# theouterlimitz/Audio-Mastering-Engine

Measured on AMD Instinct MI355X. Metric: mastered Msamples/sec (48 kHz stereo f32) at 1/2/4/8 GPUs; % HBM roofline, higher is better.
Workload: dtype f64

## Files before the change

### audio-mastering-engine_amd/csrc/amx_dyn.hip

```cpp
#include "amx_dev.hpp"

namespace amx {

typedef double d2v __attribute__((ext_vector_type(2)));
typedef uint32_t u4v __attribute__((ext_vector_type(4)));

#define AMX_TAB 32769

#define AMX_RMS_N 4096
#define AMX_RMS_MAXLOOK 1024

__device__ __forceinline__ int rms_slot(int k) { return k + (k >> 4); }

__device__ __forceinline__ uint32_t rms_floor(uint64_t S, uint32_t cnt, double rc) {
    const double sd = fma((double)(uint32_t)(S >> 32), 4294967296.0, (double)(uint32_t)S);
    const double cd = (double)cnt;
    const uint32_t k = (uint32_t)__builtin_amdgcn_sqrtf((float)(sd * rc));
    const uint32_t k1 = k + 1;
    const bool up = (double)__umul24(k1, k1) * cd <= sd;
    const bool down = (double)__umul24(k, k) * cd > sd;
    const uint32_t r = k + (uint32_t)up - (uint32_t)(down & !up);
    return cnt ? (r > 32768u ? 32768u : r) : 0u;
}

#ifndef AMX_RMS_N256
#define AMX_RMS_N256 4096
#endif
template <int LP, int N>
__global__ void __launch_bounds__(AMX_BLOCK) k_rms(const ChainDev *__restrict__ cdp,
                                                   const ChunkDev *__restrict__ chunks,
                                                   const uint32_t *__restrict__ bands,
                                                   uint16_t *__restrict__ mi, int64_t nloc,
                                                   int *bact) {
    constexpr int F = N - LP;
    constexpr int PER = N / AMX_BLOCK;
    constexpr int VEC = PER / 4;
    static_assert(F % AMX_BLOCK == 0 && PER % 4 == 0, "tile shape");
    __shared__ unsigned long long P[N + N / 16];
    __shared__ unsigned long long wsum[AMX_BLOCK / 64];
    const int look = cdp->look;
    const int c = blockIdx.y, b = blockIdx.z;
    const ChunkDev ch = chunks[c];
    const int64_t base = (int64_t)blockIdx.x * F;
    if (base >= ch.n) return;
    const uint32_t *x = bands + b * nloc + ch.loc_off;
    uint16_t *mo = mi + b * nloc + ch.loc_off;
    const int64_t rowlen = (ch.n + 15) / 16 * 16;
    const int64_t f0 = base - LP;
    const int t = threadIdx.x;
    uint32_t v[PER];
    if (f0 >= 0 && f0 + N <= ch.n) {
#pragma unroll
        for (int q = 0; q < VEC; q++) {
            const u4v u = *reinterpret_cast<const u4v *>(x + f0 + t * PER + 4 * q);
#pragma unroll
            for (int e = 0; e < 4; e++) {
                const int32_t a0 = lo16(u[e]), a1 = hi16(u[e]);
                v[4 * q + e] = (uint32_t)(a0 * a0) + (uint32_t)(a1 * a1);
            }
        }
    } else {
#pragma unroll
        for (int q = 0; q < VEC; q++) {
            const int64_t f = f0 + t * PER + 4 * q;
            const bool ok = f >= 0 && f < rowlen;
            const u4v u = *reinterpret_cast<const u4v *>(x + (ok ? f : 0));
#pragma unroll
            for (int e = 0; e < 4; e++) {
                const int32_t a0 = lo16(u[e]), a1 = hi16(u[e]);
                v[4 * q + e] = (ok && f + e < ch.n) ? (uint32_t)(a0 * a0) + (uint32_t)(a1 * a1) : 0u;
            }
        }
    }
    unsigned long long run = 0;
#pragma unroll
    for (int q = 0; q < PER; q++) run += v[q];
    unsigned long long incl = run;
    const int lane = t & 63, w = t >> 6;
#pragma unroll
    for (int o = 1; o < 64; o <<= 1) {
        const unsigned long long up = __shfl_up(incl, o);
        if (lane >= o) incl += up;
    }
    if (lane == 63) wsum[w] = incl;
    __syncthreads();
    unsigned long long p = incl - run;
    for (int q = 0; q < w; q++) p += wsum[q];
    const int s0 = rms_slot(t * PER);
#pragma unroll
    for (int q = 0; q < PER; q++) { p += v[q]; P[s0 + q] = p; }
    __syncthreads();
    constexpr int OUT = F / AMX_BLOCK;
    const uint32_t cfull = 2u * (uint32_t)look;
    const double rfull = 1.0 / (double)cfull;
    const bool whole = base >= look && base + F <= ch.n;
    auto rms_at = [&](int k) -> uint32_t {
        const uint32_t nn = (uint32_t)t + (uint32_t)k * AMX_BLOCK;
        const uint32_t e1 = nn + (LP - 1), e0 = e1 - (uint32_t)look;
        const uint64_t S = P[e1 + (e1 >> 4)] - P[e0 + (e0 >> 4)];
        if (whole) return rms_floor(S, cfull, rfull);
        const int64_t i = base + nn;
        const bool head = i < look;
        const uint32_t cnt = head ? 2u * (uint32_t)i : cfull;
        return rms_floor(S, cnt, head ? 1.0 / (double)cnt : rfull);
    };
    const uint32_t rq = (uint32_t)cdp->rq[b];
    bool hot = false;
    if (whole) {
#pragma unroll
        for (int k = 0; k < OUT; k++) {
            const uint32_t rms = rms_at(k);
            hot |= rms >= rq;
            mo[base + t + k * AMX_BLOCK] = (uint16_t)rms;
        }
    } else {
#pragma unroll
        for (int k = 0; k < OUT; k++) {
            const int64_t i = base + t + k * AMX_BLOCK;
            const uint32_t rms = rms_at(k);
            hot |= i < ch.n && rms >= rq;
            if (i < rowlen) mo[i] = i < ch.n ? (uint16_t)rms : (uint16_t)0;
        }
    }
    if (__syncthreads_or(hot) && t == 0 && bact[b] == 0) bact[b] = 1;
}

__device__ __forceinline__ double m_of(const double *__restrict__ mt, uint32_t r) {
    return mt[r < 32768u ? r : 32768u];
}


template <bool RCP>
__device__ __forceinline__ double env_div(double m, double a, double ra) {
    if constexpr (RCP) {
        const double q = m * ra;
        return fma(fma(-q, a, m), ra, q);
    } else {
        return m / a;
    }
}

__device__ __forceinline__ double min_f64_raw(double a, double b) {
    double r;
    asm("v_min_f64 %0, %1, %2" : "=v"(r) : "v"(a), "v"(b));
    return r;
}

__device__ __forceinline__ double env_step3(double att, double m, double inc, double dec) {
    const double up = min_f64_raw(att + inc, m);
    const double dn = fmax(att - dec, 0.0);
    return att <= m ? up : dn;
}

template <bool RCP>
__device__ __forceinline__ double env_step(const ChainDev &cd, double att, double m) {
    return env_step3(att, m, env_div<RCP>(m, cd.env_A, cd.env_rA), env_div<RCP>(m, cd.env_R, cd.env_rR));
}

__device__ __forceinline__ int mul16(int v, double f) {
    return (int)floor((double)v * f);
}

__device__ __forceinline__ double exp10_gain(const double *__restrict__ E, double x) {
    const double k = rint(x * E[0]);
    double r = fma(E[1], k, x);
    r = fma(E[2], k, r);
    double u = r * E[3];
    u = fma(E[4], r, u);
    double p = fma(E[5], u, E[6]);
#pragma unroll
    for (int i = 7; i < 15; i++) p = fma(u, p, E[i]);
    p = fma(u, p, 1.0);
    p = fma(u, p, 1.0);
    return ldexp(p, (int)k);
}

__device__ __forceinline__ double gain_factor(const ChainDev &cd, double att) {
    const double q = -att * cd.exc[15];
    return exp10_gain(cd.exc, fma(fma(-q, 20.0, -att), cd.exc[15], q));
}

__device__ __forceinline__ uint32_t gain_apply(uint32_t v, double f) {
    return pack2((int16_t)mul16(lo16(v), f), (int16_t)mul16(hi16(v), f));
}

__device__ __forceinline__ uint32_t gain_frame(const ChainDev &cd, uint32_t v, double att) {
    return gain_apply(v, gain_factor(cd, att));
}

#define AMX_ENV_TF_ 16

__device__ __forceinline__ double lane_val(double v, int i) {
    const long long x = __double_as_longlong(v);
    const int lo = __builtin_amdgcn_readlane((int)x, i);
    const int hi = __builtin_amdgcn_readlane((int)(x >> 32), i);
    return __longlong_as_double(((long long)hi << 32) | (unsigned)lo);
}

template <bool RCP>
__device__ double env_rerun_wave(const ChainDev &cd, const uint16_t *m, const double *mt, double *ckr,
                                 int64_t f0, int64_t f1, double ns, double old_end) {
    __shared__ __attribute__((aligned(16))) double s_m[64], s_i[64], s_d[64];
    const int lane = threadIdx.x & 63;
    const bool ckl = (lane & (AMX_ENV_TF_ - 1)) == 0;
    double c = ns;
    auto ridx = [&](int64_t f) -> uint32_t { return f < f1 ? (uint32_t)m[f] : 0xffffffffu; };
    auto gath = [&](uint32_t r) -> double { return r == 0xffffffffu ? 0.0 : m_of(mt, r); };
    auto ckld = [&](int64_t f) -> double { return ckl && f < f1 ? ckr[f / AMX_ENV_TF_] : 0.0; };
    double ml = gath(ridx(f0 + lane));
    uint32_t ib = ridx(f0 + 128 + lane);
    double m1 = gath(ridx(f0 + 64 + lane));
    double ol = ckld(f0 + lane), o1 = ckld(f0 + 64 + lane);
    for (int64_t base = f0; base < f1; base += 64) {
        const uint32_t ic = ridx(base + 192 + lane);
        const double m2 = gath(ib);
        const double o2 = ckld(base + 128 + lane);
        s_m[lane] = ml;
        s_i[lane] = env_div<RCP>(ml, cd.env_A, cd.env_rA);
        s_d[lane] = env_div<RCP>(ml, cd.env_R, cd.env_rR);
        __builtin_amdgcn_fence(__ATOMIC_SEQ_CST, "wavefront");
        __builtin_amdgcn_wave_barrier();
        double mine = c;
        int stop = 4;
#pragma unroll
        for (int t = 0; t < 4; t++) {
            double mv[16], iv[16], dv[16];
#pragma unroll
            for (int q = 0; q < 16; q += 2) {
                const d2v a = *reinterpret_cast<const d2v *>(s_m + 16 * t + q);
                const d2v b = *reinterpret_cast<const d2v *>(s_i + 16 * t + q);
                const d2v d = *reinterpret_cast<const d2v *>(s_d + 16 * t + q);
                mv[q] = a.x; mv[q + 1] = a.y;
                iv[q] = b.x; iv[q + 1] = b.y;
                dv[q] = d.x; dv[q + 1] = d.y;
            }
            const bool same = base + 16 * t < f1 && c == lane_val(ol, 16 * t);
            if (__builtin_amdgcn_readfirstlane((int)same)) { stop = t; break; }
            mine = lane == 16 * t ? c : mine;
#pragma unroll
            for (int q = 0; q < 16; q++) c = env_step3(c, mv[q], iv[q], dv[q]);
        }
        __builtin_amdgcn_wave_barrier();
        if (ckl && (lane >> 4) < stop && base + lane < f1) ckr[(base + lane) / AMX_ENV_TF_] = mine;
        if (stop < 4) return old_end;
        ml = m1;
        m1 = m2;
        ib = ic;
        ol = o1;
        o1 = o2;
    }
    return c;
}

struct EnvBands {
    int mask;
    int nb;
    __device__ __forceinline__ bool act(int b) const { return (mask >> b) & 1; }
};
__device__ __forceinline__ EnvBands env_bands(const int *bact) {
    EnvBands e;
    e.mask = 0;
#pragma unroll
    for (int b = 0; b < 3; b++) e.mask |= (__builtin_amdgcn_readfirstlane(bact[b]) != 0) << b;
    e.nb = __builtin_popcount(e.mask);
    return e;
}
__device__ __forceinline__ int env_slot_band(const EnvBands &e, int s) {
    int m = e.mask;
    for (int k = 0; k < s; k++) m &= m - 1;
    return __builtin_ctz(m | 8);
}

#define AMX_ENV_TF 16
#define AMX_ENV_MP 18
#define AMX_ENV_PF 8

typedef uint32_t u2v __attribute__((ext_vector_type(2)));

__device__ __forceinline__ void env_gather(const double *__restrict__ mt, const u2v (&I)[4],
                                           double (&G)[16]) {
#pragma unroll
    for (int i = 0; i < 4; i++) {
#pragma unroll
        for (int e = 0; e < 4; e++) {
            const uint32_t r = (I[i][e >> 1] >> (16 * (e & 1))) & 0xffffu;
            G[4 * i + e] = mt[r];
        }
    }
}

template <bool RCP>
__device__ __forceinline__ void env0_tile(const ChainDev &cd, double *sm, double (&G)[16],
                                          u2v (&Islot)[4], const u2v (&Inext)[4],
                                          const uint16_t *const (&irow)[4], const double *mt, int q,
                                          int ntile, int nwarm, int64_t start, int64_t end,
                                          double *ckr, double &att, double &s_spec, bool &any) {
    const int lane = threadIdx.x & 63;
#pragma unroll
    for (int i = 0; i < 4; i++) {
        double *d = sm + ((lane >> 2) + 16 * i) * AMX_ENV_MP + 4 * (lane & 3);
        *reinterpret_cast<d2v *>(d) = d2v{G[4 * i], G[4 * i + 1]};
        *reinterpret_cast<d2v *>(d + 2) = d2v{G[4 * i + 2], G[4 * i + 3]};
    }
    __builtin_amdgcn_wave_barrier();
    {
        const int qn = (q + AMX_ENV_PF < ntile ? q + AMX_ENV_PF : q) * AMX_ENV_TF;
#pragma unroll
        for (int i = 0; i < 4; i++) Islot[i] = *reinterpret_cast<const u2v *>(irow[i] + qn);
        env_gather(mt, Inext, G);
    }
    const int64_t f0 = start + (int64_t)q * AMX_ENV_TF;
    const bool in = f0 >= 0 && f0 < end;
    double mv[AMX_ENV_TF];
#pragma unroll
    for (int i = 0; i < 8; i++) {
        const d2v v = *reinterpret_cast<const d2v *>(sm + lane * AMX_ENV_MP + 2 * i);
        mv[2 * i] = v.x;
        mv[2 * i + 1] = v.y;
    }
    __builtin_amdgcn_wave_barrier();
    if (q == nwarm) s_spec = att;
    if (in) {
        if (q >= nwarm) {
            ckr[f0 / AMX_ENV_TF] = att;
            uint32_t h = 0, l = 0;
#pragma unroll
            for (int f = 0; f < AMX_ENV_TF; f++) {
                const unsigned long long x = (unsigned long long)__double_as_longlong(mv[f]);
                h |= (uint32_t)(x >> 32);
                l |= (uint32_t)x;
            }
            any |= ((h & 0x7fffffffu) | l) != 0u;
        }
        double iv[AMX_ENV_TF], dv[AMX_ENV_TF];
#pragma unroll
        for (int f = 0; f < AMX_ENV_TF; f++) {
            iv[f] = env_div<RCP>(mv[f], cd.env_A, cd.env_rA);
            dv[f] = env_div<RCP>(mv[f], cd.env_R, cd.env_rR);
        }
#pragma unroll
        for (int f = 0; f < AMX_ENV_TF; f++) att = env_step3(att, mv[f], iv[f], dv[f]);
    }
}

#define AMX_ENV_WG 4
#define AMX_ENV_LDS_PIN (48 * 1024)
template <bool RCP>
__global__ void __launch_bounds__(64 * AMX_ENV_WG) k_env0(const ChainDev *__restrict__ cdp,
                                             const ChunkDev *__restrict__ chunks,
                                             const SegDev *__restrict__ es, int n_es,
                                             const uint16_t *__restrict__ mi,
                                             const double *__restrict__ tabs,
                                             double *__restrict__ ck,
                                             double *__restrict__ sv, double *__restrict__ ev,
                                             int *__restrict__ act, int64_t nloc, int warm,
                                             int *__restrict__ flags) {
    __shared__ __attribute__((aligned(16))) double sm_all[AMX_ENV_WG][64 * AMX_ENV_MP];
    const ChainDev &cd = *cdp;
    const int lane = threadIdx.x & 63, wv = __builtin_amdgcn_readfirstlane(threadIdx.x >> 6);
    double *sm = sm_all[wv];
    if (blockIdx.x == 0 && blockIdx.y == 0 && threadIdx.x < AMX_ENV_MAX_ROUNDS) flags[threadIdx.x] = 0;
    if (blockIdx.x == 0 && blockIdx.y == 0 && threadIdx.x < 64) {
        for (int k = lane; k < AMX_ENV_MAX_ROUNDS * AMX_ENV_NCTR; k += 64) flags[AMX_ENV_MAX_ROUNDS + k] = 0;
        if (lane < 3) flags[AMX_ENV_LIST + lane] = 0;
    }
    const EnvBands eb = env_bands(flags + AMX_ENV_BACT);
    if ((int)blockIdx.y >= eb.nb) return;
    const int b = env_slot_band(eb, blockIdx.y);
    es += cd.etab[eb.nb].es_off;
    n_es = cd.etab[eb.nb].n_es;
    const int Le = cd.etab[eb.nb].Le, ld = cd.es_ld;
    if ((int)(blockIdx.x * (blockDim.x >> 6)) * 64 >= n_es) return;
    const int j = (blockIdx.x * (blockDim.x >> 6) + wv) * 64 + lane;
    const bool valid = j < n_es;
    const SegDev sg = es[valid ? j : n_es - 1];
    const ChunkDev ch = chunks[sg.chunk];
    const int64_t rowoff = b * nloc + ch.loc_off;
    const int64_t start = sg.pos - warm;
    const int64_t end = valid ? sg.pos + sg.len : sg.pos;
    double *ckr = ck + rowoff / AMX_ENV_TF;
    const double *mt = tabs + (int64_t)b * 3 * AMX_TAB;
    const int ntile = (warm + Le) / AMX_ENV_TF, nwarm = warm / AMX_ENV_TF;
    const uint16_t *irow[4];
#pragma unroll
    for (int i = 0; i < 4; i++) {
        const int r = 16 * i + (lane >> 2);
        irow[i] = mi + __shfl(rowoff + start, r) + 4 * (lane & 3);
    }
    u2v I[AMX_ENV_PF][4];
#pragma unroll
    for (int u = 0; u < AMX_ENV_PF; u++)
#pragma unroll
        for (int i = 0; i < 4; i++) I[u][i] = *reinterpret_cast<const u2v *>(irow[i] + u * AMX_ENV_TF);
    double G[2][16];
    env_gather(mt, I[0], G[0]);
    env_gather(mt, I[1], G[1]);
    double att = 0.0, s_spec = 0.0;
    if (cd.env_guess && start >= 0) att = mt[mi[rowoff + start]];
    bool any = false;
    for (int q0 = 0; q0 < ntile; q0 += AMX_ENV_PF) {
#pragma unroll
        for (int u = 0; u < AMX_ENV_PF; u++)
            env0_tile<RCP>(cd, sm, G[u & 1], I[u], I[(u + 2) % AMX_ENV_PF], irow, mt,
                           q0 + u, ntile, nwarm, start, end, ckr, att, s_spec, any);
    }
    if (valid) {
        sv[(int64_t)b * ld + j] = s_spec;
        ev[(int64_t)b * ld + j] = att;
        act[(int64_t)b * ld + j] = any ? 1 : 0;
    }
}

template <bool RCP>
__device__ __forceinline__ double env_fix_segment(const ChainDev &cd, const uint16_t *mrow,
                                                  const double *mt, double *ckr, int64_t pos, int len,
                                                  bool active, double ns, double old_end) {
    if (!active) {
        const int64_t k0 = pos / AMX_ENV_TF_, k1 = (pos + len + AMX_ENV_TF_ - 1) / AMX_ENV_TF_;
        for (int64_t k = k0 + (threadIdx.x & 63); k < k1; k += 64) ckr[k] = ns;
        return ns;
    }
    return env_rerun_wave<RCP>(cd, mrow, mt, ckr, pos, pos + len, ns, old_end);
}

template <bool RCP>
__global__ void __launch_bounds__(64) k_envneed(const ChainDev *__restrict__ cdp,
                                                const SegDev *__restrict__ es, int n_es,
                                                const double *__restrict__ sv,
                                                const double *__restrict__ ev,
                                                const int *__restrict__ act, int *flags,
                                                int *__restrict__ prev, int *__restrict__ list) {
    const ChainDev &cd = *cdp;
    const int b = blockIdx.y, lane = threadIdx.x;
    const EnvBands eb = env_bands(flags + AMX_ENV_BACT);
    if (!eb.act(b)) return;
    es += cd.etab[eb.nb].es_off;
    n_es = cd.etab[eb.nb].n_es;
    const int w0 = blockIdx.x * 64;
    if (w0 >= n_es) return;
    const int j = w0 + lane;
    const bool valid = j < n_es;
    const int64_t bo = (int64_t)b * cd.es_ld;
    const SegDev sg = es[valid ? j : n_es - 1];
    const bool a = valid && act[bo + j] != 0;
    const unsigned long long am = __ballot(a);
    const unsigned long long below = lane ? am & (~0ull >> (64 - lane)) : 0ull;
    int p = below ? w0 + 63 - __clzll((long long)below) : -1;
    if (p < sg.first) p = -1;
    const bool lb = valid && p < 0 && sg.first < w0;
    if (__ballot(lb)) {
        const int first0 = __shfl(sg.first, 0);
        int last = -1;
        for (int base = w0 - 64; base + 63 >= first0; base -= 64) {
            const int jj = base + lane;
            const unsigned long long mk = __ballot(jj >= first0 && act[bo + jj] != 0);
            if (mk) { last = base + 63 - __clzll((long long)mk); break; }
        }
        if (lb) p = last;
    }
    bool need = false;
    if (valid) {
        prev[bo + j] = p;
        need = !((p >= 0 ? ev[bo + p] : 0.0) == sv[bo + j]);
    }
    const unsigned long long nm = __ballot(need);
    if (nm) {
        int base = 0;
        if (lane == 0) base = atomicAdd(flags + AMX_ENV_LIST, __popcll(nm));
        base = __shfl(base, 0);
        const unsigned long long lt = lane ? ~0ull >> (64 - lane) : 0ull;
        if (need) list[base + __popcll(nm & lt)] = (int)(bo + j);
    }
}

template <bool RCP>
__global__ void __launch_bounds__(64) k_envwide(const ChainDev *__restrict__ cdp,
                                                const ChunkDev *__restrict__ chunks,
                                                const SegDev *__restrict__ es,
                                                const uint16_t *__restrict__ mm,
                                                const double *__restrict__ tabs,
                                                double *__restrict__ ck, double *sv, double *ev,
                                                const int *__restrict__ act, int *flags,
                                                const int *__restrict__ prev,
                                                const int *__restrict__ list, int64_t nloc) {
    const int count = __builtin_amdgcn_readfirstlane(flags[AMX_ENV_LIST]);
    if (blockIdx.x == 0 && threadIdx.x == 0) flags[AMX_ENV_MAX_ROUNDS + 3] = count;
    if ((int)blockIdx.x >= count) return;
    const ChainDev &cd = *cdp;
    const int lane = threadIdx.x;
    const EnvBands eb = env_bands(flags + AMX_ENV_BACT);
    const SegDev *et = es + cd.etab[eb.nb].es_off;
    const int ld = cd.es_ld;
    for (int i = blockIdx.x; i < count; i += gridDim.x) {
        const int k = __builtin_amdgcn_readfirstlane(list[i]);
        const int b = k / ld, j = k - b * ld;
        const int64_t bo = (int64_t)b * ld;
        const SegDev sg = et[j];
        const int p = prev[bo + j];
        const double ns = p >= 0 ? ev[bo + p] : 0.0;
        const int64_t ro = b * nloc + chunks[sg.chunk].loc_off;
        const double r = env_fix_segment<RCP>(cd, mm + ro, tabs + (int64_t)b * 3 * AMX_TAB, ck + ro / AMX_ENV_TF_,
                                              sg.pos, sg.len, act[bo + j] != 0, ns, ev[bo + j]);
        __builtin_amdgcn_wave_barrier();
        if (lane == 0) {
            sv[bo + j] = ns;
            ev[bo + j] = r;
        }
    }
}

#ifndef AMX_ENV_CHAIN_WAVES
#define AMX_ENV_CHAIN_WAVES 2048
#endif
template <bool RCP>
__global__ void __launch_bounds__(64) k_envheads(const ChainDev *__restrict__ cdp,
                                                 const SegDev *__restrict__ es, int n_es,
                                                 const double *__restrict__ sv,
                                                 const double *__restrict__ ev,
                                                 int *flags, int *__restrict__ list,
                                                 int *__restrict__ hmark) {
    const ChainDev &cd = *cdp;
    const int b = blockIdx.y, lane = threadIdx.x;
    const EnvBands eb = env_bands(flags + AMX_ENV_BACT);
    if (!eb.act(b)) return;
    es += cd.etab[eb.nb].es_off;
    n_es = cd.etab[eb.nb].n_es;
    if ((int)blockIdx.x * 64 >= n_es) return;
    const int j = blockIdx.x * 64 + lane;
    const int64_t bo = (int64_t)b * cd.es_ld;
    bool head = false;
    if (j < n_es) {
        const int first = es[j].first;
        const bool need = !(sv[bo + j] == (j == first ? 0.0 : ev[bo + j - 1]));
        bool needp = false;
        if (j > first) needp = !(sv[bo + j - 1] == (j - 1 == first ? 0.0 : ev[bo + j - 2]));
        head = need && !needp;
        hmark[bo + j] = head ? 1 : 0;
    }
    const unsigned long long hm = __ballot(head);
    if (hm) {
        int base = 0;
        if (lane == 0) base = atomicAdd(flags + AMX_ENV_LIST + 1, __popcll(hm));
        base = __shfl(base, 0);
        const unsigned long long below = lane ? hm & (~0ull >> (64 - lane)) : 0ull;
        if (head) list[base + __popcll(below)] = (int)(bo + j);
    }
}

template <bool RCP>
__global__ void __launch_bounds__(64) k_envchain(const ChainDev *__restrict__ cdp,
                                                 const ChunkDev *__restrict__ chunks,
                                                 const SegDev *__restrict__ es,
                                                 const uint16_t *__restrict__ mm,
                                                 const double *__restrict__ tabs,
                                                 double *__restrict__ ck, double *sv, double *ev,
                                                 const int *__restrict__ act, int *flags,
                                                 const int *__restrict__ list,
                                                 const int *__restrict__ hmark, int64_t nloc) {
    const int count = __builtin_amdgcn_readfirstlane(flags[AMX_ENV_LIST + 1]);
    if ((int)blockIdx.x >= count) return;
    const ChainDev &cd = *cdp;
    const int lane = threadIdx.x;
    const EnvBands eb = env_bands(flags + AMX_ENV_BACT);
    const SegDev *et = es + cd.etab[eb.nb].es_off;
    const int ld = cd.es_ld;
    int *ctr = flags + AMX_ENV_MAX_ROUNDS;
    int runs = 0, longest = 0, chains = 0;
    bool stale = false;
    const int n_es = cd.etab[eb.nb].n_es;
    for (int i = blockIdx.x; i < count; i += gridDim.x) {
        const int k = __builtin_amdgcn_readfirstlane(list[i]);
        const int b = k / ld, j = k - b * ld;
        const int64_t bo = (int64_t)b * ld;
        const double *mt = tabs + (int64_t)b * 3 * AMX_TAB;
        SegDev sg = et[j];
        const int64_t ro = b * nloc + chunks[sg.chunk].loc_off;
        double *ckr = ck + ro / AMX_ENV_TF_;
        double state = j == sg.first ? 0.0 : ev[bo + j - 1];
        int cur = j, walked = 0;
        bool done = false;
        while (!done) {
            const bool a = act[bo + cur] != 0;
            double old_end = ev[bo + cur];
            const double r = env_fix_segment<RCP>(cd, mm + ro, mt, ckr, sg.pos, sg.len, a, state, old_end);
            walked++;
            __builtin_amdgcn_wave_barrier();
            if (lane == 0) {
                sv[bo + cur] = state;
                ev[bo + cur] = r;
            }
            if (sg.last) break;
            int nx = cur + 1;
            while (true) {
                const int kk = nx + lane;
                const bool inch = kk < n_es && et[kk < n_es ? kk : n_es - 1].first == sg.first;
                bool hk = false, ak = false, st = true;
                double svk = 0.0, evk = 0.0;
                if (inch) {
                    hk = hmark[bo + kk] != 0;
                    ak = act[bo + kk] != 0;
                    svk = sv[bo + kk];
                    evk = ev[bo + kk];
                    st = hk || ak || svk == r;
                }
                const unsigned long long mk = __ballot(st);
                const int f = mk ? __ffsll((long long)mk) - 1 : 64;
                if (f > 0) {
                    const SegDev s0 = et[nx], s1 = et[nx + f - 1];
                    const int64_t k0 = s0.pos / AMX_ENV_TF_, k1 = (s1.pos + s1.len + AMX_ENV_TF_ - 1) / AMX_ENV_TF_;
                    for (int64_t q = k0 + lane; q < k1; q += 64) ckr[q] = r;
                    if (lane < f) {
                        sv[bo + kk] = r;
                        ev[bo + kk] = r;
                    }
                    old_end = __shfl(evk, f - 1);
                    walked += f;
                }
                if (f == 64) {
                    nx += 64;
                    continue;
                }
                const bool ins = __shfl((int)inch, f) != 0, hs = __shfl((int)hk, f) != 0;
                const double ss = __shfl(svk, f);
                if (!ins) { done = true; break; }
                if (hs) {
                    stale = stale || !(r == old_end);
                    done = true;
                    break;
                }
                if (ss == r) { done = true; break; }
                state = r;
                cur = nx + f;
                sg = et[cur];
                break;
            }
        }
        runs += walked;
        longest = walked > longest ? walked : longest;
        chains++;
    }
    if (lane == 0) {
        if (stale) flags[AMX_ENV_LIST + 2] = 1;
        atomicAdd(ctr + 0, runs);
        atomicMax(ctr + 1, longest);
        atomicAdd(ctr + 2, chains);
    }
}

template <bool RCP>
__global__ void __launch_bounds__(64) k_envseq(const ChainDev *__restrict__ cdp,
                                               const ChunkDev *__restrict__ chunks,
                                               const SegDev *__restrict__ es, int n_es,
                                               const int *__restrict__ eseg0,
                                               const int *__restrict__ neseg,
                                               const uint16_t *__restrict__ mm,
                                               const double *__restrict__ tabs,
                                               double *__restrict__ ck,
// ... 431 lines not shown
```

### audio-mastering-engine_amd/csrc/amx_plan.cpp

```cpp
#include "../../include/amx.h"
#include "amx_internal.hpp"

#include <algorithm>
#include <climits>
#include <cmath>
#include <cstdio>
#include <cstdarg>
#include <cstdlib>
#include <cstring>
#include <string>
#include <vector>

namespace {

thread_local std::string g_err;

int fail(int code, const char *fmt, ...) {
    char buf[512];
    va_list ap;
    va_start(ap, fmt);
    vsnprintf(buf, sizeof buf, fmt, ap);
    va_end(ap);
    g_err = buf;
    return code;
// ... 428 lines not shown
    cd.fs = fs;
    p->mono16 = (desc->input_s16 && desc->channels_in == 1) ? 1 : 0;
    cd.chin = p->mono16 ? 2 : desc->channels_in;
    cd.in_s16 = desc->input_s16 ? 1 : 0;
    cd.analog_on = desc->analog_on ? 1 : 0;
    cd.has_lut = desc->tanh_lut ? 1 : 0;
    cd.drive = desc->analog_drive;
    for (int k = 0; k < 6; k++) {
        cd.an_lo[k] = desc->analog_lo_ba[k];
        cd.an_hi[k] = desc->analog_hi_ba[k];
    }
    cd.an_glo1 = desc->analog_lo_gain - 1.0;
    cd.an_ghi1 = desc->analog_hi_gain - 1.0;
    int mask = 0, D = 0;
    for (int s = 0; s < 4; s++) {
        int kind = desc->eq_kind[s];
        int want = (s == 0 || s == 3) ? 1 : 2;
        if (kind != 0 && kind != want) {
            delete p;
            return fail(AMX_EINVAL, "eq stage %d: kind %d not supported at this position", s, kind);
        }
        EqStageDev &st = cd.st[s];
        st.kind = kind;
        if (!kind) continue;
        mask |= 1 << s;
        D += kind == 1 ? 2 : 8;
        st.neg = desc->eq_gain_db[s] < 0 ? 1 : 0;
        st.g = desc->eq_gain[s];
        st.gm1 = desc->eq_gain[s] - 1.0;
        st.gf = (float)desc->eq_gain[s];
        for (int k = 0; k < 24; k++) st.c[k] = desc->eq_coef[s][k];
    }
    {
        int c = 0;
        for (int s = 0; s < 4; s++) {
            const EqStageDev &st = cd.st[s];
            if (!st.kind) continue;
            const double *k = st.c;
            int nsec = st.kind == 1 ? 1 : 4;
            for (int q = 0; q < nsec; q++) {
                cd.eqc[c++] = k[6 * q + 0];
                cd.eqc[c++] = k[6 * q + 1];
                cd.eqc[c++] = k[6 * q + 2];
                cd.eqc[c++] = k[6 * q + 4];
                cd.eqc[c++] = k[6 * q + 5];
            }
            if (st.kind == 2) cd.eqc[c++] = st.gm1;
            else if (!st.neg) cd.eqc[c++] = st.gm1;
            else {
                const bool first = (mask & ((1 << s) - 1)) == 0;
                cd.eqc[c++] = first ? (double)st.gf : st.g;
            }
        }
    }
    cd.eq_mask = mask;
    cd.eq_dim = D;
    p->mask = mask;
    p->D = D;
    cd.width_on = desc->width_on ? 1 : 0;
    cd.width = desc->width;
    cd.mb_on = p->mb = desc->multiband_on ? 1 : 0;
    for (int k = 0; k < 12; k++) {
        cd.xlo[k] = desc->xover_lo_sos[k];
        cd.xhi[k] = desc->xover_hi_sos[k];
    }
    cd.look = (int32_t)(5.0 * (fs / 1000.0));
    {
        double f0 = 1681.974450955533, G = 3.999843853973347, Q = 0.7071752369554196;
        double K = std::tan(M_PI * f0 / (double)kfs);
        double Vh = std::pow(10.0, G / 20.0);
        double Vb = std::pow(Vh, 0.4996667741545416);
        double pb[3] = {0.0, 0.0, 0.0}, pa[3] = {1.0, 0.0, 0.0};
        double rb[3] = {1.0, -2.0, 1.0}, ra[3] = {1.0, 0.0, 0.0};
        double a0 = 1.0 + K / Q + K * K;
        pb[0] = (Vh + Vb * K / Q + K * K) / a0;
        pb[1] = 2.0 * (K * K - Vh) / a0;
        pb[2] = (Vh - Vb * K / Q + K * K) / a0;
        pa[1] = 2.0 * (K * K - 1.0) / a0;
        pa[2] = (1.0 - K / Q + K * K) / a0;
        f0 = 38.13547087602444;
        Q = 0.5003270373238773;
        K = std::tan(M_PI * f0 / (double)kfs);
        ra[1] = 2.0 * (K * K - 1.0) / (1.0 + K / Q + K * K);
        ra[2] = (1.0 - K / Q + K * K) / (1.0 + K / Q + K * K);
        for (int k = 0; k < 3; k++) {
            cd.kw1[k] = pb[k];
            cd.kw1[3 + k] = pa[k];
            cd.kw2[k] = rb[k];
            cd.kw2[3 + k] = ra[k];
        }
        p->kdf_b[0] = pb[0] * rb[0];
        p->kdf_b[1] = pb[0] * rb[1] + pb[1] * rb[0];
        p->kdf_b[2] = pb[0] * rb[2] + pb[1] * rb[1] + pb[2] * rb[0];
        p->kdf_b[3] = pb[1] * rb[2] + pb[2] * rb[1];
        p->kdf_b[4] = pb[2] * rb[2];
        p->kdf_a[0] = pa[0] * ra[0];
        p->kdf_a[1] = pa[0] * ra[1] + pa[1] * ra[0];
        p->kdf_a[2] = pa[0] * ra[2] + pa[1] * ra[1] + pa[2] * ra[0];
        p->kdf_a[3] = pa[1] * ra[2] + pa[2] * ra[1];
        p->kdf_a[4] = pa[2] * ra[2];
    }
    std::vector<double> tabs;
    if (p->mb) {
        tabs.assign((size_t)3 * 3 * 32769, 0.0);
        const double A = 5.0 * (fs / 1000.0), R = 50.0 * (fs / 1000.0);
        for (int b = 0; b < 3; b++) {
            double thr = 32768.0 * std::pow(10.0, desc->comp_threshold_db[b] / 20.0);
            double ratio = desc->comp_ratio[b];
            if (ratio == 0.0) {
                delete p;
                return fail(AMX_EINVAL, "compressor ratio must be non-zero");
            }
            int rthr = 0;
            while (rthr <= 32768 && !((double)rthr > thr)) rthr++;
            cd.rthr[b] = rthr;
            double k = 1.0 - (1.0 / ratio);
            double ln10 = std::log(10.0);
            double *mt = &tabs[(size_t)b * 3 * 32769];
            for (int r = 0; r <= 32768; r++) {
                double m;
                if (desc->comp_m_table[b]) {
                    m = desc->comp_m_table[b][r];
                } else {
                    double over = 0.0;
                    if (r != 0) {
                        double db = 20 * (std::log((double)r / thr) / ln10);
                        over = (0 > db) ? 0.0 : db;
                    }
                    m = k * over;
                }
                mt[r] = m;
                mt[32769 + r] = m / A;
                mt[2 * 32769 + r] = m / R;
            }
            int rq = 0;
            while (rq <= 32768 && mt[rq] == 0.0) rq++;
            cd.rq[b] = rq;
        }
        {
            static const double exc[16] = {
                0x1.a934f0979a371p+1, -0x1.34413509f79ffp-2, 0x1.9dc1da994fd21p-59,
                -0x1.f48ad494ea3e9p-53, 0x1.26bb1bbb55516p+1, 0x1.ade156a5dcb37p-26,
                0x1.28af3fca7ab0cp-22, 0x1.71dee623fde64p-19, 0x1.a01997c89e6b0p-16,
                0x1.a01a014761f6ep-13, 0x1.6c16c1852b7b0p-10, 0x1.1111111122322p-7,
                0x1.55555555502a1p-5, 0x1.5555555555511p-3, 0x1.000000000000bp-1, 0.05};
            for (int i = 0; i < 16; i++) cd.exc[i] = exc[i];
        }
        cd.env_A = A;
        cd.env_R = R;
        cd.env_rA = 1.0 / A;
        cd.env_rR = 1.0 / R;
        cd.env_guess = 1;
        if (const char *ev = std::getenv("AMX_ENV_GUESS")) cd.env_guess = std::atoi(ev) != 0;
        cd.env_rcp = 1;
        for (size_t i = 0; i < (size_t)3 * 3 * 32769 && cd.env_rcp; i += 1) {
            if (i % (3 * 32769) >= 32769) continue;
            const double m = tabs[i];
            const double qa = m * cd.env_rA, qr = m * cd.env_rR;
            const double ca = std::fma(std::fma(-qa, A, m), cd.env_rA, qa);
            const double cr = std::fma(std::fma(-qr, R, m), cd.env_rR, qr);
            if (ca != m / A || cr != m / R) cd.env_rcp = 0;
        }
    }
    int n_tracks = 0;
    for (int c = 0; c < n_chunks; c++) {
        if (chunks[c].frames < 0 || chunks[c].in_offset < 0 || chunks[c].track < 0) {
            delete p;
            return fail(AMX_EINVAL, "chunk %d: negative field", c);
        }
        if (c > 0 && chunks[c].track < chunks[c - 1].track) {
            delete p;
            return fail(AMX_EINVAL, "chunks must be ordered by track");
        }
        n_tracks = chunks[c].track + 1 > n_tracks ? chunks[c].track + 1 : n_tracks;
    }
    p->n_tracks = n_tracks;
    p->n_chunks = n_chunks;
    if (p->mb) {
        int wg = 2;
        if (const char *ev = std::getenv("AMX_ENV_WG")) wg = std::atoi(ev);
        int64_t le_min = 1024;
        if (const char *ev = std::getenv("AMX_ENV_LEMIN")) le_min = std::max(128, std::atoi(ev)) / 128 * 128;
        if (wg > 0) {
            p->env_wg = std::min(wg, 4);
            p->env_pin = 1;
            if (!env_le) {
                int dev = 0, ncu = 0;
                if (hipGetDevice(&dev) != hipSuccess ||
                    hipDeviceGetAttribute(&ncu, hipDeviceAttributeMultiprocessorCount, dev) != hipSuccess || ncu < 3)
                    ncu = 256;
                int bandtab = 1;
                if (const char *ev = std::getenv("AMX_ENV_BANDTAB")) bandtab = std::atoi(ev);
                int64_t total = 0;
                for (int c = 0; c < n_chunks; c++) total += chunks[c].frames;
                for (int t = 3; t >= 1; t--) {
                    const int64_t fit = (int64_t)(ncu / t) * 64 * p->env_wg;
                    int64_t lo = (t == 3 || std::getenv("AMX_ENV_LEMIN")) ? le_min : 512;
                    if (const char *ev = std::getenv("AMX_ENV_LEMIN2"))
                        if (t < 3) lo = std::max(128, std::atoi(ev)) / 128 * 128;
                    int64_t Le = std::max<int64_t>(lo, (total / fit + 127) / 128 * 128);
                    for (;; Le += 128) {
                        int64_t ne = 0;
                        for (int c = 0; c < n_chunks; c++) ne += (chunks[c].frames + Le - 1) / Le;
                        if (ne <= fit || Le >= (int64_t)1 << 24) break;
                    }
                    p->Le_t[t] = (t == 3 || bandtab) ? (int)Le : p->Le_t[3];
                }
                p->Le = p->Le_t[3];
            }
        }
        for (int t = 1; t <= 3; t++)
            if (p->Le_t[t] == 0) p->Le_t[t] = p->Le;
        if (desc->env_warm_frames < 0 && p->Le_t[3] <= 16384) p->warm = 1536;
    }
    int64_t loc = 0, outo = 0;
    p->spans.assign(n_tracks, SpanDev{});
    std::vector<int> track_seen(n_tracks, 0);
    for (int c = 0; c < n_chunks; c++) {
        ChunkDev ch{};
        ch.in_off = chunks[c].in_offset;
        ch.loc_off = loc;
        ch.out_off = outo;
        ch.n = chunks[c].frames;
        int64_t n1 = ch.n, n2 = ch.n;
        if (p->mb && ch.n > 0) {
            n1 = overlay_len(ch.n, fs);
            n2 = overlay_len(n1, fs);
        }
        ch.out_n = n2;
        ch.track = chunks[c].track;
        p->in_frames = std::max(p->in_frames, (int64_t)(chunks[c].in_offset + chunks[c].frames));
        ch.seg0 = (int32_t)p->segs.size();
        int64_t ns = (ch.n + p->L - 1) / p->L;
        ch.nseg = (int32_t)ns;
        add_blocks(p->blks, ch.seg0, (int32_t)ns, c);
        for (int64_t k = 0; k < ns; k++) {
            SegDev s{};
            s.pos = k * p->L;
            s.chunk = c;
            s.len = (int32_t)((ch.n - s.pos) < p->L ? (ch.n - s.pos) : p->L);
            s.first = ch.seg0;
            s.last = (k == ns - 1) ? 1 : 0;
            p->segs.push_back(s);
        }
        SpanDev &sp = p->spans[ch.track];
        if (!track_seen[ch.track]) {
            sp.out_off = outo;
            track_seen[ch.track] = 1;
        }
        sp.out_n += n2;
        p->chunks.push_back(ch);
        p->n1tab.push_back(n1);
        p->max_chunk_out = n2 > p->max_chunk_out ? n2 : p->max_chunk_out;
        p->max_chunk_n = ch.n > p->max_chunk_n ? ch.n : p->max_chunk_n;
        p->an_blocks += (ch.n + 4095) / 4096;
        if (ch.n > 0 && ((ch.in_off & 1) != 0 || ch.n < 4)) p->an_vec = 0;
        loc += (ch.n + 15) / 16 * 16;
        outo += n2;
    }
    if (loc >= ((int64_t)1 << 31) || outo >= ((int64_t)1 << 31)) {
        delete p;
        return fail(AMX_ERANGE, "a plan holds fewer than 2^31 frames (%lld): split the batch",
                    (long long)std::max(loc, outo));
    }
    p->nloc = loc;
    if (p->mb) {
        int ld = 0;
        for (int t = 3; t >= 1; t--) {
            if (t < 3 && p->Le_t[t] == p->Le_t[3]) {
                p->cd.etab[t] = p->cd.etab[3];
                continue;
            }
            const int Le = p->Le_t[t];
            const int es_off = (int)p->esegs.size(), ch_off = (int)p->eseg0.size();
            for (int c = 0; c < n_chunks; c++) {
                const int64_t n = p->chunks[c].n;
                const int64_t ne = (n + Le - 1) / Le;
                p->eseg0.push_back((int)p->esegs.size() - es_off);
                p->neseg.push_back((int)ne);
                for (int64_t k = 0; k < ne; k++) {
                    SegDev e{};
                    e.pos = k * Le;
                    e.chunk = c;
                    e.len = (int32_t)((n - e.pos) < Le ? (n - e.pos) : Le);
                    e.first = p->eseg0.back();
                    e.last = (k == ne - 1) ? 1 : 0;
                    p->esegs.push_back(e);
                }
            }
            const int n_es = (int)p->esegs.size() - es_off;
            p->cd.etab[t].es_off = es_off;
            p->cd.etab[t].n_es = n_es;
            p->cd.etab[t].ch_off = ch_off;
            p->cd.etab[t].Le = Le;
            ld = std::max(ld, n_es);
        }
        p->cd.etab[0] = p->cd.etab[3];
        p->cd.es_ld = ld;
        p->n_es = ld;
    }
    p->out_frames = outo;
    p->n_seg = (int)p->segs.size();
    const int64_t uL = p->upL, uM = p->upM, uS = p->up_src, uD = p->up_dst, uP = p->up_pc;
    auto J = [&](int64_t f) { return (f * uL + uM - 1) / uM; };
    int64_t pattern = -1;
    for (int t = 0; t < n_tracks; t++) {
        SpanDev &sp = p->spans[t];
        sp.tframe0 = track_frame0 ? track_frame0[t] : 0;
        sp.ttotal = track_total_frames ? track_total_frames[t] : sp.out_n;
        sp.kseg0 = (int32_t)p->ksegs.size();
        const int Lseg = p->resamp ? p->upLout : p->Lkw;
        const int Lsin = p->resamp ? p->upLin : p->Lkw;
        if (p->resamp && p->up_ok) {
            sp.m_tframe0 = J(sp.tframe0);
            sp.m_n = J(sp.tframe0 + sp.out_n) - sp.m_tframe0;
            sp.m_total = J(sp.ttotal);
            const int64_t pat = sp.m_tframe0 * uD - sp.tframe0 * uP * uS;
            if (sp.out_n > 0) {
                if (pattern >= 0 && pat != pattern) {
                    delete p;
                    return fail(AMX_EINVAL, "spans with different 192 kHz phase patterns in one plan");
                }
                pattern = pat;
            }
        } else {
            sp.m_tframe0 = sp.tframe0;
            sp.m_n = sp.out_n;
            sp.m_total = sp.ttotal;
        }
        sp.edge_lo = sp.tframe0 > 0 ? 1 : 0;
        sp.edge_hi = sp.tframe0 + sp.out_n < sp.ttotal ? 1 : 0;
        int64_t nk = (p->resamp && !p->up_ok) ? 0 : (sp.m_n + Lseg - 1) / Lseg;
        sp.nkseg = (int32_t)nk;
        add_blocks(p->kblks, sp.kseg0, (int32_t)nk, t);
        for (int64_t k = 0; k < nk; k++) {
            KwSegDev s{};
            s.out_pos = sp.out_off + k * Lsin;
            s.tframe = sp.m_tframe0 + k * Lseg;
            s.track = t;
            s.len = (int32_t)((sp.m_n - k * Lseg) < Lseg ? (sp.m_n - k * Lseg) : Lseg);
            s.first = sp.kseg0;
            s.last = (k == nk - 1) ? 1 : 0;
            p->ksegs.push_back(s);
        }
        p->max_span = sp.out_n > p->max_span ? sp.out_n : p->max_span;
        p->max_nkseg = sp.nkseg > p->max_nkseg ? sp.nkseg : p->max_nkseg;
        p->max_hops = std::max(p->max_hops, sp.m_total / p->hop + 1);
    }
    if (p->resamp && p->up_ok) {
        if (pattern < 0) pattern = 0;
        obase.resize(p->upLout);
        oph.resize(p->upLout);
        owt.resize(p->upLout);
        const float inv = 1.0f / (float)uS;
        for (int64_t n = 0; n < p->upLout; n++) {
            const int64_t pos = pattern + n * uD;
            const int64_t idx = pos / uS;
            obase[n] = (int32_t)(idx / uP);
            oph[n] = (int32_t)(idx % uP);
            owt[n] = (float)(pos % uS) * inv;
        }
        if (p->up_static && pattern != 0) p->up_static = 0;
        if (!p->up_static && !p->up_lin && p->up_taps == 32) {
            fcnt.assign((size_t)p->upLin, 0);
            bool ok = p->upL >= p->upM;
            for (int64_t n = 0; n < p->upLout && ok; n++) {
// ... 1331 lines not shown
```

Baseline: 31580.

## Process four envelope fix segments per wave in k_envwide with double-buffered LDS

The envelope fix-up kernel now packs four list segments into one 64-lane wave, with each 16-lane group rerunning its segment through a new double-buffered LDS staging routine instead of one wave per segment. The attack/release step drops its clamp at zero when the reciprocal path is enabled, and the host now enables that path only when R >= 1 and all table values are non-negative, which makes the clamp provably redundant. The default warm-up frame count is also reduced, trading warm-up work against a higher chance of re-fix rounds. Packing four segments per wave raises lane utilisation but adds divergence and LDS traffic per wave.

```diff
diff --git a/audio-mastering-engine_amd/csrc/amx_dyn.hip b/audio-mastering-engine_amd/csrc/amx_dyn.hip
--- a/audio-mastering-engine_amd/csrc/amx_dyn.hip
+++ b/audio-mastering-engine_amd/csrc/amx_dyn.hip
@@ -146,15 +146,16 @@
     return r;
 }
 
+template <bool POS>
 __device__ __forceinline__ double env_step3(double att, double m, double inc, double dec) {
     const double up = min_f64_raw(att + inc, m);
-    const double dn = fmax(att - dec, 0.0);
+    const double dn = POS ? att - dec : fmax(att - dec, 0.0);
     return att <= m ? up : dn;
 }
 
 template <bool RCP>
 __device__ __forceinline__ double env_step(const ChainDev &cd, double att, double m) {
-    return env_step3(att, m, env_div<RCP>(m, cd.env_A, cd.env_rA), env_div<RCP>(m, cd.env_R, cd.env_rR));
+    return env_step3<RCP>(att, m, env_div<RCP>(m, cd.env_A, cd.env_rA), env_div<RCP>(m, cd.env_R, cd.env_rR));
 }
 
 __device__ __forceinline__ int mul16(int v, double f) {
@@ -238,7 +239,7 @@
             if (__builtin_amdgcn_readfirstlane((int)same)) { stop = t; break; }
             mine = lane == 16 * t ? c : mine;
 #pragma unroll
-            for (int q = 0; q < 16; q++) c = env_step3(c, mv[q], iv[q], dv[q]);
+            for (int q = 0; q < 16; q++) c = env_step3<RCP>(c, mv[q], iv[q], dv[q]);
         }
         __builtin_amdgcn_wave_barrier();
         if (ckl && (lane >> 4) < stop && base + lane < f1) ckr[(base + lane) / AMX_ENV_TF_] = mine;
@@ -252,6 +253,86 @@
     return c;
 }
 
+template <bool RCP>
+__device__ double env_rerun_wave4(const ChainDev &cd, int mode, const uint16_t *m, const double *mt,
+                                  double *ckr, int64_t f0, int64_t f1, double ns, double old_end) {
+    __shared__ __attribute__((aligned(16))) double s_m[2][4][16], s_i[2][4][16], s_d[2][4][16];
+    const int lane = threadIdx.x & 63, g = lane >> 4, l = lane & 15;
+    if (mode == 2) {
+        const int64_t k0 = f0 / AMX_ENV_TF_, k1 = (f1 + AMX_ENV_TF_ - 1) / AMX_ENV_TF_;
+        for (int64_t k = k0 + l; k < k1; k += 16) ckr[k] = ns;
+    }
+    bool live = mode == 1 && f0 < f1;
+    double c = ns, res = ns;
+    if (!live) f1 = f0;
+    auto ridx = [&](int64_t f) -> uint32_t { return m[f < f1 ? f : f0]; };
+    auto gath = [&](uint32_t r) -> double { return m_of(mt, r); };
+    auto ckld = [&](int64_t f) -> double { return ckr[(f < f1 ? f : f0) / AMX_ENV_TF_]; };
+    auto stage = [&](int p, int64_t f, double mf) {
+        const double mv = f < f1 ? mf : 0.0;
+        s_m[p][g][l] = mv;
+        s_i[p][g][l] = env_div<RCP>(mv, cd.env_A, cd.env_rA);
+        s_d[p][g][l] = env_div<RCP>(mv, cd.env_R, cd.env_rR);
+        __builtin_amdgcn_fence(__ATOMIC_SEQ_CST, "wavefront");
+        __builtin_amdgcn_wave_barrier();
+    };
+    auto fetch = [&](int p, int h, double (&mv)[8], double (&iv)[8], double (&dv)[8]) {
+#pragma unroll
+        for (int q = 0; q < 8; q += 2) {
+            const d2v a = *reinterpret_cast<const d2v *>(&s_m[p][g][8 * h + q]);
+            const d2v b = *reinterpret_cast<const d2v *>(&s_i[p][g][8 * h + q]);
+            const d2v d = *reinterpret_cast<const d2v *>(&s_d[p][g][8 * h + q]);
+            mv[q] = a.x; mv[q + 1] = a.y;
+            iv[q] = b.x; iv[q + 1] = b.y;
+            dv[q] = d.x; dv[q + 1] = d.y;
+        }
+    };
+    int64_t base = f0;
+    const double m0 = gath(ridx(base + l));
+    double m1 = gath(ridx(base + 16 + l));
+    uint32_t ib = ridx(base + 32 + l);
+    double ol = ckld(base), o1 = ckld(base + 16);
+    double xm[8], xi[8], xd[8], ym[8], yi[8], yd[8];
+    int p = 0;
+    stage(0, base + l, m0);
+    fetch(0, 0, xm, xi, xd);
+    while (__ballot(live)) {
+        const uint32_t ic = ridx(base + 48 + l);
+        const double m2 = gath(ib);
+        const double o2 = ckld(base + 32);
+        const bool same = c == ol;
+        const bool go = live && !same;
+        if (live && same) {
+            live = false;
+            res = old_end;
+            f1 = base;
+        }
+        if (go && l == 0) ckr[base / AMX_ENV_TF_] = c;
+        fetch(p, 1, ym, yi, yd);
+        double cn = c;
+#pragma unroll
+        for (int q = 0; q < 8; q++) cn = env_step3<RCP>(cn, xm[q], xi[q], xd[q]);
+        stage(p ^ 1, base + 16 + l, m1);
+        fetch(p ^ 1, 0, xm, xi, xd);
+#pragma unroll
+        for (int q = 0; q < 8; q++) cn = env_step3<RCP>(cn, ym[q], yi[q], yd[q]);
+        if (go) {
+            c = cn;
+            if (base + 16 >= f1) {
+                live = false;
+                res = c;
+            }
+        }
+        p ^= 1;
+        base += 16;
+        m1 = m2;
+        ib = ic;
+        ol = o1;
+        o1 = o2;
+    }
+    return res;
+}
+
 struct EnvBands {
     int mask;
     int nb;
@@ -339,7 +420,7 @@
             dv[f] = env_div<RCP>(mv[f], cd.env_R, cd.env_rR);
         }
 #pragma unroll
-        for (int f = 0; f < AMX_ENV_TF; f++) att = env_step3(att, mv[f], iv[f], dv[f]);
+        for (int f = 0; f < AMX_ENV_TF; f++) att = env_step3<RCP>(att, mv[f], iv[f], dv[f]);
     }
 }
 
@@ -485,24 +566,37 @@
                                                 const int *__restrict__ list, int64_t nloc) {
     const int count = __builtin_amdgcn_readfirstlane(flags[AMX_ENV_LIST]);
     if (blockIdx.x == 0 && threadIdx.x == 0) flags[AMX_ENV_MAX_ROUNDS + 3] = count;
-    if ((int)blockIdx.x >= count) return;
+    const int nq = (count + 3) / 4;
+    if ((int)blockIdx.x >= nq) return;
     const ChainDev &cd = *cdp;
-    const int lane = threadIdx.x;
+    const int lane = threadIdx.x, g = lane >> 4;
     const EnvBands eb = env_bands(flags + AMX_ENV_BACT);
     const SegDev *et = es + cd.etab[eb.nb].es_off;
     const int ld = cd.es_ld;
-    for (int i = blockIdx.x; i < count; i += gridDim.x) {
-        const int k = __builtin_amdgcn_readfirstlane(list[i]);
+    for (int q = blockIdx.x; q < nq; q += gridDim.x) {
+        const int i = 4 * q + g;
+        const bool has = i < count;
+        const int k = has ? list[i] : 0;
         const int b = k / ld, j = k - b * ld;
         const int64_t bo = (int64_t)b * ld;
-        const SegDev sg = et[j];
-        const int p = prev[bo + j];
-        const double ns = p >= 0 ? ev[bo + p] : 0.0;
-        const int64_t ro = b * nloc + chunks[sg.chunk].loc_off;
-        const double r = env_fix_segment<RCP>(cd, mm + ro, tabs + (int64_t)b * 3 * AMX_TAB, ck + ro / AMX_ENV_TF_,
-                                              sg.pos, sg.len, act[bo + j] != 0, ns, ev[bo + j]);
+        int mode = 0;
+        double ns = 0.0, old_end = 0.0;
+        int64_t ro = 0, pos = 0;
+        int len = 0;
+        if (has) {
+            const SegDev sg = et[j];
+            const int p = prev[bo + j];
+            ns = p >= 0 ? ev[bo + p] : 0.0;
+            old_end = ev[bo + j];
+            ro = b * nloc + chunks[sg.chunk].loc_off;
+            pos = sg.pos;
+            len = sg.len;
+            mode = act[bo + j] != 0 ? 1 : 2;
+        }
+        const double r = env_rerun_wave4<RCP>(cd, mode, mm + ro, tabs + (int64_t)b * 3 * AMX_TAB,
+                                              ck + ro / AMX_ENV_TF_, pos, pos + len, ns, old_end);
         __builtin_amdgcn_wave_barrier();
-        if (lane == 0) {
+        if (has && (lane & 15) == 0) {
             sv[bo + j] = ns;
             ev[bo + j] = r;
         }
diff --git a/audio-mastering-engine_amd/csrc/amx_plan.cpp b/audio-mastering-engine_amd/csrc/amx_plan.cpp
--- a/audio-mastering-engine_amd/csrc/amx_plan.cpp
+++ b/audio-mastering-engine_amd/csrc/amx_plan.cpp
@@ -604,10 +604,11 @@
         cd.env_rR = 1.0 / R;
         cd.env_guess = 1;
         if (const char *ev = std::getenv("AMX_ENV_GUESS")) cd.env_guess = std::atoi(ev) != 0;
-        cd.env_rcp = 1;
+        cd.env_rcp = R >= 1.0 ? 1 : 0;
         for (size_t i = 0; i < (size_t)3 * 3 * 32769 && cd.env_rcp; i += 1) {
             if (i % (3 * 32769) >= 32769) continue;
             const double m = tabs[i];
+            if (!(m >= 0.0)) cd.env_rcp = 0;
             const double qa = m * cd.env_rA, qr = m * cd.env_rR;
             const double ca = std::fma(std::fma(-qa, A, m), cd.env_rA, qa);
             const double cr = std::fma(std::fma(-qr, R, m), cd.env_rR, qr);
@@ -663,7 +664,7 @@
         }
         for (int t = 1; t <= 3; t++)
             if (p->Le_t[t] == 0) p->Le_t[t] = p->Le;
-        if (desc->env_warm_frames < 0 && p->Le_t[3] <= 16384) p->warm = 1536;
+        if (desc->env_warm_frames < 0 && p->Le_t[3] <= 16384) p->warm = 1024;
     }
     int64_t loc = 0, outo = 0;
     p->spans.assign(n_tracks, SpanDev{});
```

New measurement: 31810, median of 6. No clear change (+0.7%).
